# hall-lab/speedseq

Hardware: AMD Instinct MI355X
Metric: paired reads aligned+dup-marked/sec (higher is better)
Workload: dtype int32; 1 GPU; 1000000 synthetic 2x150 bp PE pairs per GPU vs a seeded synthetic GRCh37-shaped reference of 3100 Mbp (25 contigs, order-6 Markov model of the bundled chr20 slice + 63 planted repeat families of 10..10^4 copies at 0-10% divergence = 5% of the bases; GRCh37 itself is not available offline), bwa-mem -t 16 batch boundaries; pairs_per_gpu=1000000, read_len=150, ref_bp=3099999990, records=2058655, dup_pairs=47309, dup_pairs_local_view=47309, seeds=60444408, rescues=632178, chains=9804599, sam_lines=2009191, discordant_stream_lines=29550, splitter_stream_lines=18382, dedup_scope=single GPU = whole input, sorted_merge=single GPU: bin/sambamba sort (device radix sort of the keys)

## Files before the change

speedseq_amd/csrc/k_smem2.h:

```cpp
#ifndef SSG_K_SMEM2_H
#define SSG_K_SMEM2_H
#include "ssg_dev.h"

#define SSG_S2_QWORDS 40
enum { S2_FWD = 0, S2_BWD, S2_P3F, S2_READ, S2_P1, S2_P2, S2_P3, S2_OUT, S2_FIN };
enum { S2_PEND_NONE = 0, S2_PEND_FWD, S2_PEND_BWD, S2_PEND_P3 };

struct alignas(16) ssg_pk2_t { uint64_t w0, w1; };
SSG_DEVFN ssg_pk2_t s2_pk(const ssg_intv_t &v)
{ ssg_pk2_t p; p.w0 = v.x0 | (v.x1 & 0xffffffull) << 40; p.w1 = (v.x1 >> 24) | v.x2 << 16 | v.info << 55; return p; }
SSG_DEVFN ssg_intv_t s2_unpk(const ssg_pk2_t &p)
{ ssg_intv_t v; v.x0 = p.w0 & 0xffffffffffull; v.x1 = (p.w0 >> 40) | (p.w1 & 0xffffull) << 24; v.x2 = (p.w1 >> 16) & 0x7fffffffffull; v.info = p.w1 >> 55; return v; }
SSG_DEVFN void s2_set_intv(const ssg_index_view_t &ix, int c, ssg_intv_t &ik)
{
	ik.x0 = ix.L2[c] + 1; ik.x2 = ix.L2[c+1] - ix.L2[c]; ik.x1 = ix.L2[3-c] + 1; ik.info = 0;
}

#ifdef SSG_EMU
static unsigned long long ssg_s2_stat[64];
SSG_DEVFN unsigned long long s2_wall() { return 1; }
#else
__device__ unsigned long long ssg_s2_stat[64];
SSG_DEVFN unsigned long long s2_wall() { return (unsigned long long)wall_clock64(); }
#endif
#define S2_STAT_MIN(i, v) atomicMin(&ssg_s2_stat[i], (unsigned long long)(v))
#define S2_STAT_MAX(i, v) atomicMax(&ssg_s2_stat[i], (unsigned long long)(v))
#define S2_STAT_ADD(i, v) atomicAdd(&ssg_s2_stat[i], (unsigned long long)(v))

#ifndef SSG_S2_WAVES
#define SSG_S2_WAVES 4
#endif
#ifndef SSG_S2_TRIPS
#define SSG_S2_TRIPS 2
#endif

#ifdef SSG_EMU
SSG_DEVFN int wv_uni(int v) { return v; }
SSG_DEVFN uint64_t wv_uni64(uint64_t v) { return v; }
#else
SSG_DEVFN int wv_uni(int v) { return __builtin_amdgcn_readfirstlane(v); }
SSG_DEVFN uint64_t wv_uni64(uint64_t v) { return (uint64_t)(uint32_t)__builtin_amdgcn_readfirstlane((int)(uint32_t)v) | (uint64_t)(uint32_t)__builtin_amdgcn_readfirstlane((int)(uint32_t)(v >> 32)) << 32; }
#endif
SSG_DEVFN ssg_intv_t wv_uni_intv(const ssg_intv_t &v) { ssg_intv_t o; o.x0 = wv_uni64(v.x0); o.x1 = wv_uni64(v.x1); o.x2 = wv_uni64(v.x2); o.info = wv_uni64(v.info); return o; }

SSG_DEVFN unsigned long long s2_wave_read(const ssg_index_view_t &ix, const ssg_mem_opt_t &opt, const int split_len, const int it, const int32_t *read_ids, const uint8_t *seq, const int64_t *off,
                                          ssg_intv_t *out_intv, int32_t *out_n, const int cap, uint8_t *qb, ssg_pk2_t *l0, ssg_pk2_t *l1)
{
	const int lane = wv_lane();
	unsigned long long nx = 0;
	const int r = read_ids ? read_ids[it] : it;
	const uint8_t *q = seq + off[r];
	const int len = (int)(off[r+1] - off[r]);
	ssg_wave_ldssync();
	for (int b = lane; b < len; b += 64) qb[b] = q[b];
	ssg_wave_ldssync();
	ssg_intv_t *const mem = out_intv + (long)it * cap;
	const int left = -2 - out_n[it];
	const bool skip_p3 = left >= 1;
	const int n_p3 = skip_p3 ? left - 1 : 0;
	int mem_n = n_p3, ovf = 0;
	auto smem1 = [&](const int sx, uint64_t min_intv) -> int {
		if (min_intv < 1) min_intv = 1;
		ssg_intv_t ik; s2_set_intv(ix, (int)qb[sx], ik); ik.info = (uint64_t)(sx + 1);
		int n = 0, i = sx + 1;
		bool stop = false;
		while (!stop && i < len) {
			const int cq = wv_uni((int)qb[i]);
			if (cq < 4) {
				const ssg_intv_t ok = wv_uni_intv(ssg_bwt_extend1_lean(ix, ik, 3 - cq, 0)); ++nx;
				if (ok.x2 != ik.x2) { l0[n++] = s2_pk(ik); stop = ok.x2 < min_intv; }
				if (!stop) { ik = ok; ik.info = (uint64_t)(i + 1); ++i; }
			} else { l0[n++] = s2_pk(ik); stop = true; }
		}
		if (!stop) l0[n++] = s2_pk(ik);
		const int ret = (int)ik.info;
		int cur = 0, prev_n = n, rev = 1, m1_n = 0, m1_last_beg = 0;
		bool more = true;
		for (int ib = sx - 1; more && ib >= -1; --ib) {
			const int cb = ib < 0 ? -1 : wv_uni((int)qb[ib]) < 4 ? wv_uni((int)qb[ib]) : -1;
			int curr_n = 0; bool have_last = false; uint64_t last_x2 = 0;
			ssg_wave_ldssync();
			for (int base = 0; base < prev_n; base += 64) {
				const int jj = base + lane; const bool valid = jj < prev_n;
				ssg_intv_t p; p.x0 = p.x1 = p.x2 = p.info = 0;
				if (valid) p = s2_unpk((cur ? l1 : l0)[rev ? prev_n - 1 - jj : jj]);
				ssg_intv_t okc; okc.x0 = okc.x1 = okc.x2 = okc.info = 0;
				if (valid && cb >= 0) okc = ssg_bwt_extend1_lean(ix, p, cb, 1);
				if (cb >= 0) nx += (unsigned long long)(prev_n - base < 64 ? prev_n - base : 64);
				const bool alive = valid && cb >= 0 && okc.x2 >= min_intv;
				if (base == 0 && !wv_get((int)alive, 0)) {
					const int beg = ib + 1;
					if (m1_n == 0 || beg < m1_last_beg) {
						++m1_n; m1_last_beg = beg;
						const int end0 = wv_get((int)(uint32_t)p.info, 0);
						if (end0 - beg >= opt.min_seed_len) {
							if (mem_n < cap) { if (lane == 0) { ssg_intv_t o = p; o.info |= (uint64_t)beg << 32; mem[mem_n] = o; } } else ovf = 1;
							++mem_n;
						}
					}
				}
				const unsigned long long am = wv_ballot(alive);
				if (am) {
					const unsigned long long below = am & ((1ull << lane) - 1ull);
					const int pl = below ? 63 - __clzll(below) : 0;
					const uint64_t px2 = (uint64_t)wv_shfl64_xor((long long)okc.x2, lane ^ pl);
					const bool push = alive && (below ? okc.x2 != px2 : (!have_last || okc.x2 != last_x2));
					const unsigned long long pm = wv_ballot(push);
					if (push) { ssg_intv_t o = okc; o.info = p.info; (cur ? l0 : l1)[curr_n + __popcll(pm & ((1ull << lane) - 1ull))] = s2_pk(o); }
					curr_n += __popcll(pm);
					have_last = true; last_x2 = (uint64_t)wv_get64((long long)okc.x2, 63 - __clzll(am));
				}
			}
			if (curr_n == 0) more = false;
			else { cur ^= 1; rev = 0; prev_n = curr_n; }
		}
		ssg_wave_ldssync();
		return ret;
	};
	if (len >= opt.min_seed_len) {
		int x = 0;
		while (x < len) { if (wv_uni((int)qb[x]) < 4) x = smem1(x, 1); else ++x; }
		const int old_n = mem_n < cap ? mem_n : cap;
		ssg_wave_memsync();
		for (int k = n_p3; k < old_n; ++k) {
			const ssg_intv_t m = wv_uni_intv(mem[k]);
			const int start = (int)(m.info >> 32), end = (int)(uint32_t)m.info;
			if (end - start >= split_len && m.x2 <= (uint64_t)opt.split_width) {
				const int sx = (start + end) >> 1;
				if (wv_uni((int)qb[sx]) < 4) (void)smem1(sx, m.x2 + 1);
			}
		}
		if (opt.max_mem_intv > 0 && !skip_p3) {
			x = 0;
			while (x < len) {
				if (wv_uni((int)qb[x]) > 3) ++x;
				else {
					ssg_intv_t ik; s2_set_intv(ix, (int)qb[x], ik);
					int i = x + 1, nxt = len; bool stop = false;
					while (!stop && i < len) {
						const int cq = wv_uni((int)qb[i]);
						if (cq < 4) {
							const ssg_intv_t ok = wv_uni_intv(ssg_bwt_extend1_lean(ix, ik, 3 - cq, 0)); ++nx;
							if (ok.x2 < (uint64_t)opt.max_mem_intv && i - x >= opt.min_seed_len) {
								if (ok.x2 > 0) {
									if (mem_n < cap) { if (lane == 0) { ssg_intv_t o = ok; o.info = (uint64_t)x << 32 | (uint64_t)(i + 1); mem[mem_n] = o; } } else ovf = 1;
									++mem_n;
								}
								nxt = i + 1; stop = true;
							} else { ik = ok; ++i; }
						} else { nxt = i + 1; stop = true; }
					}
					x = nxt;
				}
			}
		}
	}
	if (lane == 0) out_n[it] = ovf ? -1 : mem_n;
	return nx;
}

SSG_DEVFN long s2_ktab_off(int j) { return (long)(((1ull << (2 * j)) - 4ull) / 3ull); }
__global__ void ssg_k_ktab_level(ssg_index_view_t ix, int j, ssg_pk2_t *tab)
{
	const long p = (long)blockIdx.x * blockDim.x + threadIdx.x;
	if (p >= (1L << (2 * (j - 1)))) return;
	ssg_pk2_t *const out = tab + s2_ktab_off(j) + 4 * p;
	ssg_intv_t ok[4];
	if (j == 1) { for (int c = 0; c < 4; ++c) s2_set_intv(ix, c, ok[c]); }
	else ssg_bwt_extend(ix, s2_unpk(tab[s2_ktab_off(j - 1) + p]), ok, 1);
	for (int c = 0; c < 4; ++c) { ok[c].info = 0; out[c] = s2_pk(ok[c]); }
}
__global__ void ssg_k_ktab_verify(ssg_index_view_t ix, int j, long stride, const ssg_pk2_t *tab, unsigned long long *bad)
{
	const long t = (long)blockIdx.x * blockDim.x + threadIdx.x, code = t * stride;
	if (code >= (1L << (2 * j))) return;
	ssg_intv_t ik;
	s2_set_intv(ix, (int)(code & 3), ik);
	for (int k = 1; k < j; ++k) ik = ssg_bwt_extend1_lean(ix, ik, 3 - (int)((code >> (2 * k)) & 3), 0);
	const ssg_intv_t e = s2_unpk(tab[s2_ktab_off(j) + code]);
	if (ik.x2 != e.x2 || (ik.x2 && (ik.x0 != e.x0 || ik.x1 != e.x1))) atomicAdd(&bad[j], 1ull);
}
SSG_DEVFN uint64_t s2_window(const uint32_t *qw, int stride, int b)
{
	const int w0 = b >> 3, sh = (b & 7) << 2;
	const int w1 = w0 + 1 < SSG_S2_QWORDS ? w0 + 1 : SSG_S2_QWORDS - 1, w2 = w0 + 2 < SSG_S2_QWORDS ? w0 + 2 : SSG_S2_QWORDS - 1;
	uint64_t v = ((uint64_t)qw[w0 * stride] | (uint64_t)qw[w1 * stride] << 32) >> sh;
	if (sh) v |= (uint64_t)qw[w2 * stride] << (64 - sh);
	return v;
}
SSG_DEVFN uint32_t s2_code(const uint32_t *qw, int stride, int b, int n)
{
	uint64_t v = s2_window(qw, stride, b);
	v &= 0x3333333333333333ull; v = (v | v >> 2) & 0x0f0f0f0f0f0f0f0full; v = (v | v >> 4) & 0x00ff00ff00ff00ffull;
	v = (v | v >> 8) & 0x0000ffff0000ffffull; v = (v | v >> 16) & 0xffffffffull;
	return (uint32_t)v & ((1u << (2 * n)) - 1u);
}

template <bool TUNE, bool KT>
__global__ void __launch_bounds__(64, SSG_S2_WAVES) ssg_k_smem2(ssg_index_view_t ix, ssg_mem_opt_t opt, int n_reads, const int32_t *read_ids,
                           const uint8_t *seq, const int64_t *off, ssg_intv_t *out_intv, int32_t *out_n, int cap,
                           ssg_pk2_t *scratch, int scap, unsigned long long *n_extend, unsigned int *next_read, unsigned int max_ext, int max_row, uint32_t *n_ext_read, int32_t *heavy_ids, unsigned int *n_heavy,
                           const ssg_pk2_t *kt_tab, int kt_k )
{
	__shared__ uint32_t qlds[SSG_S2_QWORDS * 64];
	const long gt = (long)blockIdx.x * blockDim.x + threadIdx.x;
	const int lane = (int)(threadIdx.x & 63);
	ssg_pk2_t *const vec0 = scratch + (gt >> 6) * 2 * scap * 64 + lane, *const vec1 = vec0 + (long)scap * 64;
	const uint32_t *const ql_ = qlds + lane;
#define S2Q(i) ((int)((ql_[((i) >> 3) * 64] >> (((i) & 7) << 2)) & 15u))
#define S2V(v, e) ((v)[(long)(e) * 64])
	const int split_len = (int)(opt.min_seed_len * opt.split_factor + .499);
	unsigned long long my_nx = 0;
	unsigned int rd_nx = 0, nx_p3 = 0;
	long it = 0;
	int state = S2_READ, pend = S2_PEND_NONE;
	int len = 0, x = 0, k = 0, old_n = 0, caller = 0, mem_n = 0, ovf = 0, heavy = 0, n_p3 = -1;
	ssg_intv_t *mem = 0;
	int sx = 0, i = 0, j = 0, curr_n = 0, prev_n = 0, prev_rev = 0, flip = 0, m1_n = 0, m1_last_beg = 0, ret = 0, e_c = 0;
	uint64_t min_intv = 1, last_x2 = 0;
	ssg_intv_t ik, p;
	ik.x0 = ik.x1 = ik.x2 = ik.info = 0; p = ik;
	ssg_pk2_t pn, c0, first; pn.w0 = pn.w1 = 0; c0 = first = pn;
	if (TUNE) S2_STAT_MIN(0, s2_wall());
#define S2_FWDEND() do { ret = (int)ik.info; flip ^= 1; prev_n = curr_n < scap ? curr_n : scap; prev_rev = 1; curr_n = 0; i = sx - 1; j = 0; first = s2_pk(ik); state = S2_BWD; if (prev_n > max_row) { heavy = 1; state = S2_OUT; } } while (0)
#define S2_P3END() do { n_p3 = mem_n; nx_p3 = rd_nx; x = 0; state = S2_P1; } while (0)
#define S2_P3START() do { \
		while (x < len && S2Q(x) > 3) ++x; \
		if (x >= len) S2_P3END(); \
		else if (!KT || kt_k < 2) { s2_set_intv(ix, S2Q(x), ik); i = x + 1; state = S2_P3F; } \
		else { \
			const unsigned long long nm_ = s2_window(ql_, 64, x) & 0x4444444444444444ull; \
			int run_ = nm_ ? (int)((__ffsll(nm_) - 1) >> 2) : 16; \
			run_ = run_ > len - x ? len - x : run_; \
			if (run_ >= kt_k) { ik = s2_unpk(kt_tab[s2_ktab_off(kt_k) + (long)s2_code(ql_, 64, x, kt_k)]); i = x + kt_k; my_nx += (unsigned long long)(kt_k - 1); rd_nx += (unsigned int)(kt_k - 1); state = S2_P3F; } \
			else { my_nx += (unsigned long long)(run_ - 1); rd_nx += (unsigned int)(run_ - 1); if (x + run_ >= len) S2_P3END(); else { x += run_ + 1; state = S2_P3; } } \
		} \
	} while (0)
#define S2_RET() do { if (caller == 1) { x = ret; state = S2_P1; } else { ++k; state = S2_P2; } } while (0)
#define S2_EMIT(pp, beg) do { if (m1_n == 0 || (beg) < m1_last_beg) { ++m1_n; m1_last_beg = (beg); \
		if ((int)(uint32_t)(pp).info - (beg) >= opt.min_seed_len) { ssg_intv_t o_ = (pp); o_.info |= (uint64_t)(beg) << 32; if (mem_n < cap) mem[mem_n] = o_; else ovf = 1; ++mem_n; } } } while (0)
	for (;;) {
		SSG_UNROLL for (int trip = 0; trip < SSG_S2_TRIPS; ++trip) if ((trip == 0 || wv_ballot(pend == S2_PEND_NONE && state != S2_FIN)) && pend == S2_PEND_NONE && state != S2_FIN) {
			ssg_pk2_t *const curr = flip ? vec1 : vec0;
			if (state == S2_FWD) {
				if (i < len && S2Q(i) < 4) { pend = S2_PEND_FWD; e_c = 3 - S2Q(i); }
				else { if (curr_n < scap) S2V(curr, curr_n) = s2_pk(ik); else ovf = 1; ++curr_n; S2_FWDEND(); }
			} else if (state == S2_BWD) {
				if (j >= prev_n) {
					bool back_to_caller = curr_n == 0;
					if (!back_to_caller) { flip ^= 1; prev_n = curr_n < scap ? curr_n : scap; prev_rev = 0; curr_n = 0; j = 0; --i; first = c0; back_to_caller = i < -1; }
					if (back_to_caller) S2_RET();
				} else {
					p = s2_unpk(j == 0 ? first : pn);
					const int cb = i < 0 ? -1 : S2Q(i) < 4 ? S2Q(i) : -1;
					if (cb >= 0) { pend = S2_PEND_BWD; e_c = cb; }
					else {
						if (j == 0) S2_EMIT(p, i + 1);
						j = prev_n;
					}
				}
			} else if (state == S2_P3F) {
				if (i >= len) S2_P3END();
				else if (S2Q(i) < 4) { pend = S2_PEND_P3; e_c = 3 - S2Q(i); }
				else { x = i + 1; S2_P3START(); }
			} else if (state == S2_READ) {
				it = (long)atomicAdd(next_read, 1u);
				if (it >= n_reads) { state = S2_FIN; if (TUNE) S2_STAT_MIN(1, s2_wall()); }
				else {
					const int r = read_ids ? read_ids[it] : (int)it;
					const uint8_t *q = seq + off[r];
					len = (int)(off[r+1] - off[r]);
					mem = out_intv + (long)it * cap; mem_n = 0; ovf = 0; rd_nx = 0; nx_p3 = 0; heavy = 0;
					const unsigned al = (unsigned)((uintptr_t)q & 7), sh8 = al << 3;
					const uint64_t *const qa = (const uint64_t*)(q - al);
					const int nw = (len + 7) >> 3, nb = (int)al + len;
					for (int w0 = 0; w0 < nw; w0 += 4) {
						uint64_t t[5];
						SSG_UNROLL for (int jj = 0; jj < 5; ++jj) t[jj] = (w0 + jj) * 8 < nb ? qa[w0 + jj] : 0;
						SSG_UNROLL for (int jj = 0; jj < 4; ++jj) {
							const int w = w0 + jj;
							if (w < nw) {
								uint64_t v = sh8 ? (t[jj] >> sh8) | (t[jj + 1] << (64 - sh8)) : t[jj];
								v &= 0x0f0f0f0f0f0f0f0full;
								v = (v | v >> 4) & 0x00ff00ff00ff00ffull;
								v = (v | v >> 8) & 0x0000ffff0000ffffull;
								uint32_t v32 = (uint32_t)(v | v >> 16);
								const int nv = len - w * 8;
								if (nv < 8) v32 &= (1u << (nv << 2)) - 1u;
								qlds[w * 64 + lane] = v32;
							}
						}
					}
					x = 0;
					n_p3 = opt.max_mem_intv > 0 ? -1 : 0;
					state = len < opt.min_seed_len ? S2_OUT : opt.max_mem_intv > 0 ? S2_P3 : S2_P1;
				}
			} else if (state == S2_P1) {
				if (x >= len) { old_n = mem_n < cap ? mem_n : cap; k = n_p3 > 0 ? n_p3 : 0; state = S2_P2; }
				else if (S2Q(x) > 3) ++x;
				else { sx = x; min_intv = 1; caller = 1; state = S2_FWD; m1_n = 0; curr_n = 0; i = sx + 1; s2_set_intv(ix, S2Q(sx), ik); ik.info = (uint64_t)(sx + 1); }
			} else if (state == S2_P2) {
				if (k >= old_n) state = S2_OUT;
				else {
					const ssg_intv_t m = mem[k];
					const int start = (int)(m.info >> 32), end = (int)(uint32_t)m.info;
					if (end - start < split_len || m.x2 > (uint64_t)opt.split_width) ++k;
					else {
						sx = (start + end) >> 1; min_intv = m.x2 + 1; caller = 2; m1_n = 0; curr_n = 0; i = sx + 1;
						if (S2Q(sx) > 3) S2_RET();
						else { s2_set_intv(ix, S2Q(sx), ik); ik.info = (uint64_t)(sx + 1); state = S2_FWD; }
					}
				}
			} else if (state == S2_P3) {
				S2_P3START();
			} else {
				const bool given_up = heavy != 0;
				out_n[it] = ovf ? -1 : given_up ? (n_p3 < 0 ? -2 : -3 - n_p3) : mem_n;
				if (given_up && !ovf && heavy_ids) heavy_ids[atomicAdd(n_heavy, 1u)] = (int32_t)it;
				if (given_up) my_nx -= n_p3 < 0 ? rd_nx : rd_nx - nx_p3;
				if (n_ext_read) n_ext_read[it] = rd_nx;
				if (TUNE) { S2_STAT_ADD(8 + (64 - __clzll((unsigned long long)(rd_nx | 1u))), 1); if (given_up) S2_STAT_ADD(3, 1); }
				state = S2_READ;
			}
		}
		if (TUNE) { const unsigned long long rdy = wv_ballot(pend != S2_PEND_NONE), alv = wv_ballot(state != S2_FIN); if (lane == 0) { S2_STAT_ADD(48, 1); S2_STAT_ADD(49, __popcll(rdy)); S2_STAT_ADD(50, __popcll(alv)); } }
		if (!wv_ballot(state != S2_FIN)) break;
		const int pat_b = pend == S2_PEND_BWD ? i : pend == S2_PEND_FWD ? sx : x, pat_n = (pend == S2_PEND_BWD ? (int)p.info : i + 1) - pat_b;
		const bool by_table = KT && pend != S2_PEND_NONE && pat_n <= kt_k;
		const bool any_tab = KT && wv_ballot(by_table) != 0, any_ext = !KT || wv_ballot(pend != S2_PEND_NONE && !by_table) != 0;
		if (pend != S2_PEND_NONE) {
			const ssg_pk2_t *const prev = flip ? vec0 : vec1;
			ssg_pk2_t *const curr = flip ? vec1 : vec0;
			const bool back = pend == S2_PEND_BWD;
			const int jn = back && j + 1 < prev_n ? j + 1 : 0;
			ssg_pk2_t pf; pf.w0 = pf.w1 = 0;
			if (jn) pf = S2V(prev, prev_rev ? prev_n - 1 - jn : jn);
			ssg_intv_t okc; okc.x0 = okc.x1 = okc.x2 = okc.info = 0;
			if (any_tab) { if (by_table) okc = s2_unpk(kt_tab[s2_ktab_off(pat_n) + (long)s2_code(ql_, 64, pat_b, pat_n)]); }
			if (any_ext) { if (!by_table) okc = ssg_bwt_extend1_lean(ix, back ? p : ik, e_c, back); }
			++my_nx; ++rd_nx;
			if (pend == S2_PEND_FWD) {
				bool fwd_end = false;
				if (okc.x2 != ik.x2) {
					if (curr_n < scap) S2V(curr, curr_n) = s2_pk(ik); else ovf = 1;
					++curr_n;
					if (okc.x2 < min_intv) { S2_FWDEND(); fwd_end = true; }
				}
				if (!fwd_end) { ik = okc; ik.info = (uint64_t)(i + 1); ++i; }
			} else if (back) {
				pn = pf;
				if (okc.x2 < min_intv) { if (curr_n == 0) S2_EMIT(p, i + 1); }
				else if (curr_n == 0 || okc.x2 != last_x2) {
					ssg_intv_t o = okc; o.info = p.info;
					const ssg_pk2_t po = s2_pk(o);
					if (curr_n == 0) c0 = po;
					if (curr_n < scap) S2V(curr, curr_n) = po; else ovf = 1;
					++curr_n; last_x2 = okc.x2;
				}
				++j;
			} else {
				if (okc.x2 < (uint64_t)opt.max_mem_intv && i - x >= opt.min_seed_len) {
					if (okc.x2 > 0) { ssg_intv_t o = okc; o.info = (uint64_t)x << 32 | (uint64_t)(i + 1); if (mem_n < cap) mem[mem_n] = o; else ovf = 1; ++mem_n; }
					x = i + 1; S2_P3START();
				} else { ik = okc; ++i; }
			}
			pend = S2_PEND_NONE;
			if (rd_nx > max_ext) { heavy = 1; state = S2_OUT; }
		}
	}
	if (TUNE) S2_STAT_MAX(2, s2_wall());
#undef S2Q
#undef S2V
#undef S2_FWDEND
#undef S2_P3START
#undef S2_P3END
#undef S2_RET
#undef S2_EMIT
	if (n_extend && my_nx) atomicAdd(n_extend, my_nx);
}

#ifdef SSG_HEAVY_MIN_WAVES
#define SSG_HEAVY_BOUNDS __launch_bounds__(64, SSG_HEAVY_MIN_WAVES)
#else
#define SSG_HEAVY_BOUNDS __launch_bounds__(64)
#endif
template <int SC>
__global__ void SSG_HEAVY_BOUNDS ssg_k_smem_heavy(ssg_index_view_t ix, ssg_mem_opt_t opt, const int32_t *ids, const unsigned int *n_ids, const int32_t *read_ids,
                           const uint8_t *seq, const int64_t *off, ssg_intv_t *out_intv, int32_t *out_n, int cap, unsigned long long *n_extend, unsigned int *next)
{
	__shared__ uint8_t qb[328];
	__shared__ ssg_pk2_t lst[2][SC];
	const int split_len = (int)(opt.min_seed_len * opt.split_factor + .499);
	const int n_todo = (int)*n_ids;
	unsigned long long nx = 0;
	for (;;) {
		const long t = wv_queue_pop(next);
		if (t >= n_todo) break;
		nx += s2_wave_read(ix, opt, split_len, ids[t], read_ids, seq, off, out_intv, out_n, cap, qb, lst[0], lst[1]);
	}
	if (n_extend && nx && wv_lane() == 0) atomicAdd(n_extend, nx);
}
__global__ void ssg_k_sa_verify(ssg_index_view_t ix, int new_intv, const uint64_t *sa_new, long n_new, long stride, unsigned long long *bad)
{
	const long j = ((long)blockIdx.x * blockDim.x + threadIdx.x) * stride;
	if (j >= n_new) return;
	const uint64_t r = (uint64_t)j * (uint64_t)new_intv;
	const uint64_t want = (r % (uint64_t)ix.sa_intv) == 0 ? ix.sa[r / (uint64_t)ix.sa_intv] : ssg_bwt_sa(ix, r);
	if (sa_new[j] != want) atomicAdd(bad, 1ull);
}
#endif
```

speedseq_amd/csrc/ssg_seed.cpp:

```cpp
#include <algorithm>
#include "ssg_rt.h"
#include "k_smem2.h"
#include "../../include/ssgpu.h"
#include "ssg_index_int.h"

SSG_ABI_FP_DEFINE(seed)
static int env_int(const char *name, int dflt) { const char *e = getenv(name); return e && *e ? atoi(e) : dflt; }
static int budget_row(unsigned int max_ext) { return max_ext < 0x7fffffffu ? env_int("SSG_SMEM_MAX_ROW", 32) : 0x7fffffff; }

static constexpr auto ssg_k_smem2_plain = ssg_k_smem2<false, false>;
static constexpr auto ssg_k_smem2_kt = ssg_k_smem2<false, true>;
static constexpr auto ssg_k_smem2_tune = ssg_k_smem2<true, false>;
static constexpr auto ssg_k_smem2_kt_tune = ssg_k_smem2<true, true>;

extern "C" int ssg_seed_smem2(const ssg_index *idx, const ssg_mem_opt_t *opt, int n_reads, const uint8_t *d_seq, const int64_t *d_off, int max_len, int cap,
                              ssg_intv_t *d_intv, int32_t *d_n, unsigned long long *n_extend, unsigned int max_ext, uint32_t *d_n_ext_read)
{
	const int block = 64;
	const long nthreads = std::min<long>(((long)n_reads + block - 1) / block * block, 256L * env_int("SSG_SMEM_WAVES_PER_CU", 16) * 64)   ;
	const int scap = max_len + 2;
	const int kt_want = idx->ktab ? std::min(idx->ktab_k, opt->min_seed_len - 1) : 0;
	const int kt_k = kt_want >= 2 ? kt_want : 0;
	const ssg_pk2_t *const kt = kt_k ? (const ssg_pk2_t*)idx->ktab : (const ssg_pk2_t*)0;
	dbuf<ssg_pk2_t> scratch((size_t)nthreads * 2 * scap + 64);
	dbuf<unsigned int> d_next(4);
	const int max_row = budget_row(max_ext);
	const bool budget = max_ext < 0x7fffffffu;
	dbuf<int32_t> d_heavy(budget ? (size_t)n_reads : 1);
	if (!scratch.ok() || !d_next.ok() || !d_heavy.ok()) { ssg_err_msg = "device allocation failed: seeding work lists"; return SSG_ENOMEM; }
	CHK(d_next.zero());
	int32_t *const hv = budget ? d_heavy.p : (int32_t*)0;
	if (env_int("SSG_S2_TUNE", 0)) {
		unsigned long long st[64]; memset(st, 0, sizeof(st)); st[0] = st[1] = ~0ull;
#ifdef SSG_EMU
		memcpy(ssg_s2_stat, st, sizeof(st));
#else
		CHK(rt_sync()); CHK(rt_check(hipMemcpyToSymbol(HIP_SYMBOL(ssg_s2_stat), st, sizeof(st)), "hipMemcpyToSymbol"));
#endif
		if (kt) SSG_LAUNCH(ssg_k_smem2_kt_tune, nthreads / block, block, 0, idx->v, *opt, n_reads, (const int32_t*)0, d_seq, d_off, d_intv, d_n, cap, scratch.p, scap, n_extend, d_next.p, max_ext, max_row, d_n_ext_read, hv, d_next.p + 1, kt, kt_k);
		else SSG_LAUNCH(ssg_k_smem2_tune, nthreads / block, block, 0, idx->v, *opt, n_reads, (const int32_t*)0, d_seq, d_off, d_intv, d_n, cap, scratch.p, scap, n_extend, d_next.p, max_ext, max_row, d_n_ext_read, hv, d_next.p + 1, kt, kt_k);
		CHK(rt_sync());
#ifdef SSG_EMU
		memcpy(st, ssg_s2_stat, sizeof(st));
#else
		CHK(rt_check(hipMemcpyFromSymbol(st, HIP_SYMBOL(ssg_s2_stat), sizeof(st)), "hipMemcpyFromSymbol"));
#endif
		fprintf(stderr, "[ssgpu] smem2 timeline (ms): pool of reads empty at %.2f, last lane done at %.2f; %llu reads given up at %u extensions / rows of %d; rounds %llu, lanes ready %.1f, with a read %.1f of 64\n",
		        (double)(st[1] - st[0]) / 1e5, (double)(st[2] - st[0]) / 1e5, st[3], max_ext, max_row, st[48], st[48] ? (double)st[49] / st[48] : 0., st[48] ? (double)st[50] / st[48] : 0.);
		fprintf(stderr, "[ssgpu] smem2 reads by extensions (< 2^b):");
		for (int b = 1; b <= 24; ++b) if (st[8 + b]) fprintf(stderr, " b%d=%llu", b, st[8 + b]);
		fprintf(stderr, "\n");
	} else if (kt) SSG_LAUNCH(ssg_k_smem2_kt, nthreads / block, block, 0, idx->v, *opt, n_reads, (const int32_t*)0, d_seq, d_off, d_intv, d_n, cap, scratch.p, scap, n_extend, d_next.p, max_ext, max_row, d_n_ext_read, hv, d_next.p + 1, kt, kt_k);
	else SSG_LAUNCH(ssg_k_smem2_plain, nthreads / block, block, 0, idx->v, *opt, n_reads, (const int32_t*)0, d_seq, d_off, d_intv, d_n, cap, scratch.p, scap, n_extend, d_next.p, max_ext, max_row, d_n_ext_read, hv, d_next.p + 1, kt, kt_k);
	if (budget) {
		const long n_wg = std::min<long>(n_reads, 256L * env_int("SSG_SMEM_HEAVY_WAVES_PER_CU", 28));
		if (scap <= 160) SSG_LAUNCH(ssg_k_smem_heavy<160>, n_wg, block, 0, idx->v, *opt, (const int32_t*)d_heavy.p, (const unsigned int*)(d_next.p + 1), (const int32_t*)0, d_seq, d_off, d_intv, d_n, cap, n_extend, d_next.p + 2);
		else if (scap <= 264) SSG_LAUNCH(ssg_k_smem_heavy<264>, n_wg, block, 0, idx->v, *opt, (const int32_t*)d_heavy.p, (const unsigned int*)(d_next.p + 1), (const int32_t*)0, d_seq, d_off, d_intv, d_n, cap, n_extend, d_next.p + 2);
		else SSG_LAUNCH(ssg_k_smem_heavy<328>, n_wg, block, 0, idx->v, *opt, (const int32_t*)d_heavy.p, (const unsigned int*)(d_next.p + 1), (const int32_t*)0, d_seq, d_off, d_intv, d_n, cap, n_extend, d_next.p + 2);
	}
	return rt_sync();
}

extern "C" int ssg_index_build_ktab(ssg_index *ix)
{
	int lg = 0; while ((ix->v.seq_len >> (2 * (lg + 1))) != 0) ++lg;
	int K = env_int("SSG_KTAB_K", std::min(13, lg - 2));
	K = std::min(K, std::min(15, lg + 2));
	rt_free(ix->ktab); ix->ktab = 0; ix->ktab_k = 0;
	if (K < 2 || ix->v.seq_len >= (1ull << 40)) return 0;
	const size_t n_ent = (size_t)((((1ull << (2 * (K + 1))) - 4ull) / 3ull));
	ix->ktab = (uint64_t*)rt_malloc(n_ent * 16);
	if (!ix->ktab) { ssg_err_msg = "index allocation failed: table of short-pattern intervals"; return SSG_ENOMEM; }
	for (int j = 1; j <= K; ++j) { const long np = 1L << (2 * (j - 1)); SSG_LAUNCH(ssg_k_ktab_level, (np + 255) / 256, 256, 0, ix->v, j, (ssg_pk2_t*)ix->ktab); }
	CHK(rt_sync());
	if (env_int("SSG_KTAB_VERIFY", 0)) {
		dbuf<unsigned long long> d_bad(16); unsigned long long bad[16];
		if (!d_bad.ok()) { ssg_err_msg = "device allocation failed"; return SSG_ENOMEM; }
		CHK(d_bad.zero());
		for (int j = 1; j <= K; ++j) { const long np = 1L << (2 * j), stride = np > (1L << 22) ? np >> 22 : 1, nt = (np + stride - 1) / stride; SSG_LAUNCH(ssg_k_ktab_verify, (nt + 255) / 256, 256, 0, ix->v, j, stride, (const ssg_pk2_t*)ix->ktab, d_bad.p); }
		CHK(rt_sync()); CHK(d_bad.down(bad, 16));
		fprintf(stderr, "[ssgpu] table of short-pattern intervals, K = %d; entries that differ from forward extension, per level:", K);
		for (int j = 1; j <= K; ++j) fprintf(stderr, " %llu", bad[j]);
		fprintf(stderr, "\n");
	}
	ix->ktab_k = K;
	return 0;
}

extern "C" int ssg_sa_verify(const ssg_index *ix, int new_intv, const uint64_t *d_sa_new, long n_new)
{
	const long stride = n_new > (1L << 24) ? n_new >> 24 : 1, nt = (n_new + stride - 1) / stride;
	dbuf<unsigned long long> d_bad(1); unsigned long long bad = 0;
	if (!d_bad.ok()) { ssg_err_msg = "device allocation failed"; return SSG_ENOMEM; }
	CHK(d_bad.zero());
	SSG_LAUNCH(ssg_k_sa_verify, (nt + 255) / 256, 256, 0, ix->v, new_intv, d_sa_new, n_new, stride, d_bad.p);
	CHK(rt_sync()); CHK(d_bad.down(&bad, 1));
	fprintf(stderr, "[ssgpu] SA samples every %d rows: %llu of %ld checked entries differ from bwt_sa on the file's samples\n", new_intv, bad, nt);
	return 0;
}
```

Baseline: 5.500 million pairs/s.

## Shrink SMEM kernel read image, cache hot list entries in LDS, skip dead pushes

Adds a kernel variant with a 20-word read image in LDS for reads up to 160 bp, and uses the freed LDS to hold work-list entries 1-2 per lane. Pushes that are never read back are no longer stored. The scratch layout changes from lane-interleaved to contiguous per thread with padding. Tuning counters are also added. The aim is less global scratch traffic and more occupancy headroom, but the contiguous per-thread layout gives up coalesced access across lanes.

Result: no change. 5.524 million pairs/s (median of 6 runs) (+0.4%).

```diff
diff --git a/speedseq_amd/csrc/k_smem2.h b/speedseq_amd/csrc/k_smem2.h
--- a/speedseq_amd/csrc/k_smem2.h
+++ b/speedseq_amd/csrc/k_smem2.h
@@ -3,6 +3,7 @@
 #include "ssg_dev.h"
 
 #define SSG_S2_QWORDS 40
+#define SSG_S2_QSHORT 20
 enum { S2_FWD = 0, S2_BWD, S2_P3F, S2_READ, S2_P1, S2_P2, S2_P3, S2_OUT, S2_FIN };
 enum { S2_PEND_NONE = 0, S2_PEND_FWD, S2_PEND_BWD, S2_PEND_P3 };
 
@@ -17,10 +18,10 @@
 }
 
 #ifdef SSG_EMU
-static unsigned long long ssg_s2_stat[64];
+static unsigned long long ssg_s2_stat[96];
 SSG_DEVFN unsigned long long s2_wall() { return 1; }
 #else
-__device__ unsigned long long ssg_s2_stat[64];
+__device__ unsigned long long ssg_s2_stat[96];
 SSG_DEVFN unsigned long long s2_wall() { return (unsigned long long)wall_clock64(); }
 #endif
 #define S2_STAT_MIN(i, v) atomicMin(&ssg_s2_stat[i], (unsigned long long)(v))
@@ -33,6 +34,17 @@
 #ifndef SSG_S2_TRIPS
 #define SSG_S2_TRIPS 2
 #endif
+#ifndef SSG_S2_DEADSTORE
+#define SSG_S2_DEADSTORE 1
+#endif
+#ifndef SSG_S2_WINDOW
+#define SSG_S2_WINDOW 1
+#endif
+#ifndef SSG_S2_CONTIG
+#define SSG_S2_CONTIG 1
+#endif
+SSG_DEVFN int s2_hist6(int n) { return n <= 4 ? n - 1 : n <= 8 ? 4 : 5; }
+#define S2_SCAP_PAD(scap) (SSG_S2_CONTIG ? ((long)(scap) + 7) & ~7L : (long)(scap))
 
 #ifdef SSG_EMU
 SSG_DEVFN int wv_uni(int v) { return v; }
@@ -180,35 +192,48 @@
 	const ssg_intv_t e = s2_unpk(tab[s2_ktab_off(j) + code]);
 	if (ik.x2 != e.x2 || (ik.x2 && (ik.x0 != e.x0 || ik.x1 != e.x1))) atomicAdd(&bad[j], 1ull);
 }
-SSG_DEVFN uint64_t s2_window(const uint32_t *qw, int stride, int b)
+SSG_DEVFN uint64_t s2_window(const uint32_t *qw, int stride, int b, int nq)
 {
 	const int w0 = b >> 3, sh = (b & 7) << 2;
-	const int w1 = w0 + 1 < SSG_S2_QWORDS ? w0 + 1 : SSG_S2_QWORDS - 1, w2 = w0 + 2 < SSG_S2_QWORDS ? w0 + 2 : SSG_S2_QWORDS - 1;
+	const int w1 = w0 + 1 < nq ? w0 + 1 : nq - 1, w2 = w0 + 2 < nq ? w0 + 2 : nq - 1;
 	uint64_t v = ((uint64_t)qw[w0 * stride] | (uint64_t)qw[w1 * stride] << 32) >> sh;
 	if (sh) v |= (uint64_t)qw[w2 * stride] << (64 - sh);
 	return v;
 }
-SSG_DEVFN uint32_t s2_code(const uint32_t *qw, int stride, int b, int n)
-{
-	uint64_t v = s2_window(qw, stride, b);
+SSG_DEVFN uint32_t s2_code(const uint32_t *qw, int stride, int b, int n, int nq)
+{
+	uint64_t v = s2_window(qw, stride, b, nq);
 	v &= 0x3333333333333333ull; v = (v | v >> 2) & 0x0f0f0f0f0f0f0f0full; v = (v | v >> 4) & 0x00ff00ff00ff00ffull;
 	v = (v | v >> 8) & 0x0000ffff0000ffffull; v = (v | v >> 16) & 0xffffffffull;
 	return (uint32_t)v & ((1u << (2 * n)) - 1u);
 }
 
-template <bool TUNE, bool KT>
+template <bool TUNE, bool KT, int QW>
 __global__ void __launch_bounds__(64, SSG_S2_WAVES) ssg_k_smem2(ssg_index_view_t ix, ssg_mem_opt_t opt, int n_reads, const int32_t *read_ids,
                            const uint8_t *seq, const int64_t *off, ssg_intv_t *out_intv, int32_t *out_n, int cap,
                            ssg_pk2_t *scratch, int scap, unsigned long long *n_extend, unsigned int *next_read, unsigned int max_ext, int max_row, uint32_t *n_ext_read, int32_t *heavy_ids, unsigned int *n_heavy,
                            const ssg_pk2_t *kt_tab, int kt_k )
 {
-	__shared__ uint32_t qlds[SSG_S2_QWORDS * 64];
+	constexpr bool WIN = SSG_S2_WINDOW && QW < SSG_S2_QWORDS;
+	__shared__ uint32_t qlds[(QW + (WIN ? 16 : 0)) * 64];
 	const long gt = (long)blockIdx.x * blockDim.x + threadIdx.x;
 	const int lane = (int)(threadIdx.x & 63);
+#if SSG_S2_CONTIG
+	ssg_pk2_t *const vec0 = scratch + gt * 2 * S2_SCAP_PAD(scap), *const vec1 = vec0 + S2_SCAP_PAD(scap);
+#define S2V(v, e) ((v)[e])
+#else
 	ssg_pk2_t *const vec0 = scratch + (gt >> 6) * 2 * scap * 64 + lane, *const vec1 = vec0 + (long)scap * 64;
+#define S2V(v, e) ((v)[(long)(e) * 64])
+#endif
 	const uint32_t *const ql_ = qlds + lane;
 #define S2Q(i) ((int)((ql_[((i) >> 3) * 64] >> (((i) & 7) << 2)) & 15u))
-#define S2V(v, e) ((v)[(long)(e) * 64])
+	uint32_t *const win_ = qlds + QW * 64 + lane;
+#define S2W_IN(e) (WIN && (unsigned int)((e) - 1) < 2u)
+#define S2W_AT(l, e, w) win_[((((l) << 1) + (e) - 1) * 4 + (w)) * 64]
+#define S2W_LD(o, l, e) do { (o).w0 = (uint64_t)S2W_AT(l, e, 0) | (uint64_t)S2W_AT(l, e, 1) << 32; (o).w1 = (uint64_t)S2W_AT(l, e, 2) | (uint64_t)S2W_AT(l, e, 3) << 32; } while (0)
+#define S2W_ST(l, e, val) do { const ssg_pk2_t v_ = (val); S2W_AT(l, e, 0) = (uint32_t)v_.w0; S2W_AT(l, e, 1) = (uint32_t)(v_.w0 >> 32); S2W_AT(l, e, 2) = (uint32_t)v_.w1; S2W_AT(l, e, 3) = (uint32_t)(v_.w1 >> 32); } while (0)
+#define S2_PUSH(v, l, val, live) do { if (curr_n < scap) { if (!SSG_S2_DEADSTORE || (live)) { if (S2W_IN(curr_n)) S2W_ST(l, curr_n, val); else S2V(v, curr_n) = (val); } } else ovf = 1; ++curr_n; } while (0)
+	unsigned int t_fpush = 0, t_bpush = 0, t_fdead = 0, t_bdead = 0, t_rd = 0, t_rd12 = 0, t_brow[6] = { 0, 0, 0, 0, 0, 0 }, t_frow[6] = { 0, 0, 0, 0, 0, 0 };
 	const int split_len = (int)(opt.min_seed_len * opt.split_factor + .499);
 	unsigned long long my_nx = 0;
 	unsigned int rd_nx = 0, nx_p3 = 0;
@@ -222,17 +247,17 @@
 	ik.x0 = ik.x1 = ik.x2 = ik.info = 0; p = ik;
 	ssg_pk2_t pn, c0, first; pn.w0 = pn.w1 = 0; c0 = first = pn;
 	if (TUNE) S2_STAT_MIN(0, s2_wall());
-#define S2_FWDEND() do { ret = (int)ik.info; flip ^= 1; prev_n = curr_n < scap ? curr_n : scap; prev_rev = 1; curr_n = 0; i = sx - 1; j = 0; first = s2_pk(ik); state = S2_BWD; if (prev_n > max_row) { heavy = 1; state = S2_OUT; } } while (0)
+#define S2_FWDEND() do { if (TUNE) { SSG_UNROLL for (int b_ = 0; b_ < 6; ++b_) t_frow[b_] += (unsigned int)(s2_hist6(curr_n) == b_); } ret = (int)ik.info; flip ^= 1; prev_n = curr_n < scap ? curr_n : scap; prev_rev = 1; curr_n = 0; i = sx - 1; j = 0; first = s2_pk(ik); state = S2_BWD; if (prev_n > max_row) { heavy = 1; state = S2_OUT; } } while (0)
 #define S2_P3END() do { n_p3 = mem_n; nx_p3 = rd_nx; x = 0; state = S2_P1; } while (0)
 #define S2_P3START() do { \
 		while (x < len && S2Q(x) > 3) ++x; \
 		if (x >= len) S2_P3END(); \
 		else if (!KT || kt_k < 2) { s2_set_intv(ix, S2Q(x), ik); i = x + 1; state = S2_P3F; } \
 		else { \
-			const unsigned long long nm_ = s2_window(ql_, 64, x) & 0x4444444444444444ull; \
+			const unsigned long long nm_ = s2_window(ql_, 64, x, QW) & 0x4444444444444444ull; \
 			int run_ = nm_ ? (int)((__ffsll(nm_) - 1) >> 2) : 16; \
 			run_ = run_ > len - x ? len - x : run_; \
-			if (run_ >= kt_k) { ik = s2_unpk(kt_tab[s2_ktab_off(kt_k) + (long)s2_code(ql_, 64, x, kt_k)]); i = x + kt_k; my_nx += (unsigned long long)(kt_k - 1); rd_nx += (unsigned int)(kt_k - 1); state = S2_P3F; } \
+			if (run_ >= kt_k) { ik = s2_unpk(kt_tab[s2_ktab_off(kt_k) + (long)s2_code(ql_, 64, x, kt_k, QW)]); i = x + kt_k; my_nx += (unsigned long long)(kt_k - 1); rd_nx += (unsigned int)(kt_k - 1); state = S2_P3F; } \
 			else { my_nx += (unsigned long long)(run_ - 1); rd_nx += (unsigned int)(run_ - 1); if (x + run_ >= len) S2_P3END(); else { x += run_ + 1; state = S2_P3; } } \
 		} \
 	} while (0)
@@ -244,10 +269,11 @@
 			ssg_pk2_t *const curr = flip ? vec1 : vec0;
 			if (state == S2_FWD) {
 				if (i < len && S2Q(i) < 4) { pend = S2_PEND_FWD; e_c = 3 - S2Q(i); }
-				else { if (curr_n < scap) S2V(curr, curr_n) = s2_pk(ik); else ovf = 1; ++curr_n; S2_FWDEND(); }
+				else { S2_PUSH(curr, flip, s2_pk(ik), false); if (TUNE) { ++t_fpush; ++t_fdead; } S2_FWDEND(); }
 			} else if (state == S2_BWD) {
 				if (j >= prev_n) {
 					bool back_to_caller = curr_n == 0;
+					if (TUNE && !back_to_caller) { SSG_UNROLL for (int b = 0; b < 6; ++b) t_brow[b] += (unsigned int)(s2_hist6(curr_n) == b); }
 					if (!back_to_caller) { flip ^= 1; prev_n = curr_n < scap ? curr_n : scap; prev_rev = 0; curr_n = 0; j = 0; --i; first = c0; back_to_caller = i < -1; }
 					if (back_to_caller) S2_RET();
 				} else {
@@ -334,17 +360,20 @@
 			const bool back = pend == S2_PEND_BWD;
 			const int jn = back && j + 1 < prev_n ? j + 1 : 0;
 			ssg_pk2_t pf; pf.w0 = pf.w1 = 0;
-			if (jn) pf = S2V(prev, prev_rev ? prev_n - 1 - jn : jn);
+			const int pe = prev_rev ? prev_n - 1 - jn : jn;
+			if (jn) { if (S2W_IN(pe)) S2W_LD(pf, flip ^ 1, pe); else pf = S2V(prev, pe); }
+			if (TUNE && jn) { ++t_rd; t_rd12 += (unsigned int)(pe == 1 || pe == 2); }
 			ssg_intv_t okc; okc.x0 = okc.x1 = okc.x2 = okc.info = 0;
-			if (any_tab) { if (by_table) okc = s2_unpk(kt_tab[s2_ktab_off(pat_n) + (long)s2_code(ql_, 64, pat_b, pat_n)]); }
+			if (any_tab) { if (by_table) okc = s2_unpk(kt_tab[s2_ktab_off(pat_n) + (long)s2_code(ql_, 64, pat_b, pat_n, QW)]); }
 			if (any_ext) { if (!by_table) okc = ssg_bwt_extend1_lean(ix, back ? p : ik, e_c, back); }
 			++my_nx; ++rd_nx;
 			if (pend == S2_PEND_FWD) {
 				bool fwd_end = false;
 				if (okc.x2 != ik.x2) {
-					if (curr_n < scap) S2V(curr, curr_n) = s2_pk(ik); else ovf = 1;
-					++curr_n;
-					if (okc.x2 < min_intv) { S2_FWDEND(); fwd_end = true; }
+					const bool last = okc.x2 < min_intv;
+					S2_PUSH(curr, flip, s2_pk(ik), !last);
+					if (TUNE) { ++t_fpush; t_fdead += (unsigned int)last; }
+					if (last) { S2_FWDEND(); fwd_end = true; }
 				}
 				if (!fwd_end) { ik = okc; ik.info = (uint64_t)(i + 1); ++i; }
 			} else if (back) {
@@ -354,8 +383,9 @@
 					ssg_intv_t o = okc; o.info = p.info;
 					const ssg_pk2_t po = s2_pk(o);
 					if (curr_n == 0) c0 = po;
-					if (curr_n < scap) S2V(curr, curr_n) = po; else ovf = 1;
-					++curr_n; last_x2 = okc.x2;
+					if (TUNE) { ++t_bpush; t_bdead += (unsigned int)(curr_n == 0); }
+					S2_PUSH(curr, flip, po, curr_n != 0);
+					last_x2 = okc.x2;
 				}
 				++j;
 			} else {
@@ -369,8 +399,17 @@
 		}
 	}
 	if (TUNE) S2_STAT_MAX(2, s2_wall());
+	if (TUNE) {
+		S2_STAT_ADD(51, t_fpush); S2_STAT_ADD(52, t_bpush); S2_STAT_ADD(53, t_fdead); S2_STAT_ADD(54, t_bdead); S2_STAT_ADD(55, t_rd); S2_STAT_ADD(56, t_rd12);
+		SSG_UNROLL for (int b = 0; b < 6; ++b) { S2_STAT_ADD(64 + b, t_brow[b]); S2_STAT_ADD(72 + b, t_frow[b]); }
+	}
 #undef S2Q
 #undef S2V
+#undef S2_PUSH
+#undef S2W_IN
+#undef S2W_AT
+#undef S2W_LD
+#undef S2W_ST
 #undef S2_FWDEND
 #undef S2_P3START
 #undef S2_P3END
diff --git a/speedseq_amd/csrc/ssg_seed.cpp b/speedseq_amd/csrc/ssg_seed.cpp
--- a/speedseq_amd/csrc/ssg_seed.cpp
+++ b/speedseq_amd/csrc/ssg_seed.cpp
@@ -8,10 +8,14 @@
 static int env_int(const char *name, int dflt) { const char *e = getenv(name); return e && *e ? atoi(e) : dflt; }
 static int budget_row(unsigned int max_ext) { return max_ext < 0x7fffffffu ? env_int("SSG_SMEM_MAX_ROW", 32) : 0x7fffffff; }
 
-static constexpr auto ssg_k_smem2_plain = ssg_k_smem2<false, false>;
-static constexpr auto ssg_k_smem2_kt = ssg_k_smem2<false, true>;
-static constexpr auto ssg_k_smem2_tune = ssg_k_smem2<true, false>;
-static constexpr auto ssg_k_smem2_kt_tune = ssg_k_smem2<true, true>;
+static constexpr auto ssg_k_smem2_plain = ssg_k_smem2<false, false, SSG_S2_QWORDS>;
+static constexpr auto ssg_k_smem2_kt = ssg_k_smem2<false, true, SSG_S2_QWORDS>;
+static constexpr auto ssg_k_smem2_tune = ssg_k_smem2<true, false, SSG_S2_QWORDS>;
+static constexpr auto ssg_k_smem2_kt_tune = ssg_k_smem2<true, true, SSG_S2_QWORDS>;
+static constexpr auto ssg_k_smem2_plain_q20 = ssg_k_smem2<false, false, SSG_S2_QSHORT>;
+static constexpr auto ssg_k_smem2_kt_q20 = ssg_k_smem2<false, true, SSG_S2_QSHORT>;
+static constexpr auto ssg_k_smem2_tune_q20 = ssg_k_smem2<true, false, SSG_S2_QSHORT>;
+static constexpr auto ssg_k_smem2_kt_tune_q20 = ssg_k_smem2<true, true, SSG_S2_QSHORT>;
 
 extern "C" int ssg_seed_smem2(const ssg_index *idx, const ssg_mem_opt_t *opt, int n_reads, const uint8_t *d_seq, const int64_t *d_off, int max_len, int cap,
                               ssg_intv_t *d_intv, int32_t *d_n, unsigned long long *n_extend, unsigned int max_ext, uint32_t *d_n_ext_read)
@@ -22,7 +26,7 @@
 	const int kt_want = idx->ktab ? std::min(idx->ktab_k, opt->min_seed_len - 1) : 0;
 	const int kt_k = kt_want >= 2 ? kt_want : 0;
 	const ssg_pk2_t *const kt = kt_k ? (const ssg_pk2_t*)idx->ktab : (const ssg_pk2_t*)0;
-	dbuf<ssg_pk2_t> scratch((size_t)nthreads * 2 * scap + 64);
+	dbuf<ssg_pk2_t> scratch((size_t)nthreads * 2 * (size_t)S2_SCAP_PAD(scap) + 64);
 	dbuf<unsigned int> d_next(4);
 	const int max_row = budget_row(max_ext);
 	const bool budget = max_ext < 0x7fffffffu;
@@ -30,15 +34,18 @@
 	if (!scratch.ok() || !d_next.ok() || !d_heavy.ok()) { ssg_err_msg = "device allocation failed: seeding work lists"; return SSG_ENOMEM; }
 	CHK(d_next.zero());
 	int32_t *const hv = budget ? d_heavy.p : (int32_t*)0;
+	const bool q20 = max_len <= 8 * SSG_S2_QSHORT;
+	if (max_len > 8 * SSG_S2_QWORDS) { ssg_err_msg = "seeding: a read longer than the lane kernel's read image"; return SSG_EINVAL; }
+#define S2_LAUNCH(K) do { if (q20) SSG_LAUNCH(K##_q20, nthreads / block, block, 0, idx->v, *opt, n_reads, (const int32_t*)0, d_seq, d_off, d_intv, d_n, cap, scratch.p, scap, n_extend, d_next.p, max_ext, max_row, d_n_ext_read, hv, d_next.p + 1, kt, kt_k); \
+	else SSG_LAUNCH(K, nthreads / block, block, 0, idx->v, *opt, n_reads, (const int32_t*)0, d_seq, d_off, d_intv, d_n, cap, scratch.p, scap, n_extend, d_next.p, max_ext, max_row, d_n_ext_read, hv, d_next.p + 1, kt, kt_k); } while (0)
 	if (env_int("SSG_S2_TUNE", 0)) {
-		unsigned long long st[64]; memset(st, 0, sizeof(st)); st[0] = st[1] = ~0ull;
+		unsigned long long st[96]; memset(st, 0, sizeof(st)); st[0] = st[1] = ~0ull;
 #ifdef SSG_EMU
 		memcpy(ssg_s2_stat, st, sizeof(st));
 #else
 		CHK(rt_sync()); CHK(rt_check(hipMemcpyToSymbol(HIP_SYMBOL(ssg_s2_stat), st, sizeof(st)), "hipMemcpyToSymbol"));
 #endif
-		if (kt) SSG_LAUNCH(ssg_k_smem2_kt_tune, nthreads / block, block, 0, idx->v, *opt, n_reads, (const int32_t*)0, d_seq, d_off, d_intv, d_n, cap, scratch.p, scap, n_extend, d_next.p, max_ext, max_row, d_n_ext_read, hv, d_next.p + 1, kt, kt_k);
-		else SSG_LAUNCH(ssg_k_smem2_tune, nthreads / block, block, 0, idx->v, *opt, n_reads, (const int32_t*)0, d_seq, d_off, d_intv, d_n, cap, scratch.p, scap, n_extend, d_next.p, max_ext, max_row, d_n_ext_read, hv, d_next.p + 1, kt, kt_k);
+		if (kt) S2_LAUNCH(ssg_k_smem2_kt_tune); else S2_LAUNCH(ssg_k_smem2_tune);
 		CHK(rt_sync());
 #ifdef SSG_EMU
 		memcpy(st, ssg_s2_stat, sizeof(st));
@@ -50,8 +57,15 @@
 		fprintf(stderr, "[ssgpu] smem2 reads by extensions (< 2^b):");
 		for (int b = 1; b <= 24; ++b) if (st[8 + b]) fprintf(stderr, " b%d=%llu", b, st[8 + b]);
 		fprintf(stderr, "\n");
-	} else if (kt) SSG_LAUNCH(ssg_k_smem2_kt, nthreads / block, block, 0, idx->v, *opt, n_reads, (const int32_t*)0, d_seq, d_off, d_intv, d_n, cap, scratch.p, scap, n_extend, d_next.p, max_ext, max_row, d_n_ext_read, hv, d_next.p + 1, kt, kt_k);
-	else SSG_LAUNCH(ssg_k_smem2_plain, nthreads / block, block, 0, idx->v, *opt, n_reads, (const int32_t*)0, d_seq, d_off, d_intv, d_n, cap, scratch.p, scap, n_extend, d_next.p, max_ext, max_row, d_n_ext_read, hv, d_next.p + 1, kt, kt_k);
+		fprintf(stderr, "[ssgpu] smem2 work lists: pushes forward %llu (never read %llu), backward %llu (never read %llu); entries read %llu, at index 1-2 %llu\n", st[51], st[53], st[52], st[54], st[55], st[56]);
+		fprintf(stderr, "[ssgpu] smem2 lists of 1 2 3 4 5-8 9+ entries: backward rows");
+		for (int b = 0; b < 6; ++b) fprintf(stderr, " %llu", st[64 + b]);
+		fprintf(stderr, "; forward lists");
+		for (int b = 0; b < 6; ++b) fprintf(stderr, " %llu", st[72 + b]);
+		fprintf(stderr, "\n");
+	} else if (kt) S2_LAUNCH(ssg_k_smem2_kt);
+	else S2_LAUNCH(ssg_k_smem2_plain);
+#undef S2_LAUNCH
 	if (budget) {
 		const long n_wg = std::min<long>(n_reads, 256L * env_int("SSG_SMEM_HEAVY_WAVES_PER_CU", 28));
 		if (scap <= 160) SSG_LAUNCH(ssg_k_smem_heavy<160>, n_wg, block, 0, idx->v, *opt, (const int32_t*)d_heavy.p, (const unsigned int*)(d_next.p + 1), (const int32_t*)0, d_seq, d_off, d_intv, d_n, cap, n_extend, d_next.p + 2);
```
